# kit4b/kit4b

Hardware: AMD Instinct MI355X
Metric: Mreads/sec aligned (100 bp SE vs 3 Gbp .sfx) (higher is better)
Workload: dtype u64

## Files before the change

### kit4b_amd/csrc/k4_align.hip

```cpp
#include <stdlib.h>
#include <type_traits>
#include "k4_align_common.h"

#define K4_BS(nch) ((nch) >= 16 ? 128 : 256)
template <int NCH>
struct K4Lane {
  const uint64_t* rd;
  uint32_t* ded;
  const uint32_t* sup;
  const uint64_t* ent;
  uint64_t* memo;
  static constexpr int NW = NCH + 1;
  K4_DEV uint64_t word(int s, int c) const { return rd[(s * NW + c) * K4_BS(NCH)]; }
  K4_DEV uint64_t chunk_at(int s, int o) const {
    int w = o >> 5, sh = 2 * (o & 31);
    uint64_t hi = word(s, w);
    if (!sh) return hi;
    return (hi << sh) | (word(s, w + 1) >> (64 - sh));
  }
};

struct K4Probe {
  int cmp;
  int mm;
  int fm;
  bool exc;
};

#define K4_MEMO_NONE 0ull
K4_DEV uint64_t k4d_memo_pack(int kind, uint64_t pos, int mm, int fm) {
  return ((uint64_t)kind << 62) | ((uint64_t)(fm & 0x3FFF) << 48) | ((uint64_t)(mm & 0xFF) << 40) | (pos & 0xFFFFFFFFFFull);
}

template <int NCH>
K4_DEV K4Probe k4d_probe(const K4DevIndex& ix, const K4Lane<NCH>& ln, int s, int o, int cl, int len, uint64_t p) {
  K4Probe r;
  int64_t left = (int64_t)p - o;
  {
    const int64_t st = left < 0 ? 0 : left;
    const uint64_t b0 = (uint64_t)st >> ix.sup_shift, b1 = (uint64_t)(left + len - 1) >> ix.sup_shift;
    const uint64_t v = (((uint64_t)ln.sup[(b0 >> 5) + 1] << 32) | ln.sup[b0 >> 5]) >> (b0 & 31);
    r.exc = (v & ((2ull << (b1 - b0)) - 1ull)) != 0;
    if (r.exc && ix.sup_shift != K4_EXC_SHIFT) r.exc = k4d_any_exc(ix, left, left + len);
  }
  r.cmp = 0;
  r.mm = 0;
  r.fm = len;
  const uint32_t* wp = ix.ref2 + (left >> 4);
  uint32_t sh = (uint32_t)(left & 15) * 2;
  uint32_t wv[2 * NCH + 1];
  if (NCH <= 5 && len + 15 <= 32 * NCH) {
    uint32_t even[2 * NCH];
    k4d_load_words<2 * NCH>(wp, even);
#pragma unroll
    for (int j = 0; j < 2 * NCH + 1; j++) wv[j] = j < 2 * NCH ? even[j] : 0u;
  } else if (NCH <= 5 || len > 32 * (NCH / 2))
    k4d_load_words<2 * NCH + 1>(wp, wv);
  else {
    uint32_t half[NCH + 1];
    k4d_load_words<NCH + 1>(wp, half);
#pragma unroll
    for (int j = 0; j < 2 * NCH + 1; j++) wv[j] = j < NCH + 1 ? half[j] : 0u;
  }
  bool decided = false;
#pragma unroll
  for (int c = 0; c < NCH; c++) {
    if (32 * c < len) {
      uint64_t hi = ((uint64_t)wv[2 * c] << 32) | wv[2 * c + 1];
      uint64_t refc = sh ? (hi << sh) | (wv[2 * c + 2] >> (32 - sh)) : hi;
      uint64_t rdc = ln.word(s, c);
      uint64_t x = rdc ^ refc;
      const uint64_t xr = x & k4d_range_mask(0, len - 32 * c);
      r.mm += (int)k4d_mm_count(xr);
      if (xr && r.fm == len) r.fm = 32 * c + (__clzll(xr) >> 1);
      uint64_t cm = k4d_range_mask(o - 32 * c, o + cl - 32 * c);
      if (!decided && (x & cm)) {
        r.cmp = (rdc & cm) < (refc & cm) ? -1 : 1;
        decided = true;
      }
    }
  }
  return r;
}

template <int EL, int NCH, typename KT, bool CAPTURE>
K4_DEV int k4d_lcm_fast(const K4AlignArgs& a, const K4Lane<NCH>& ln, int len, int allow_mm, int cl, int core_delta,
                        const K4ReadParams& rp, int* p_inst, int* p_low, int* p_nxt, k4_hit* hits,
                        uint32_t& n_lookup, uint32_t& n_probe, uint32_t& n_cand, bool defer_deep = false) {
  const K4DevIndex& ix = a.ix;
  if (*p_inst > rp.max_hits && *p_low == 0) return K4_HR_HITINSTS;
  if (*p_inst >= 1 && *p_low == 0 && (*p_nxt - *p_low) < rp.mm_delta) return K4_HR_MMDELTA;
  K4State st;
  if (*p_inst <= 0 || *p_low < 0 || *p_nxt < 0) {
    st.inst = *p_inst = 0;
    st.low = *p_low = allow_mm + rp.mm_delta + 1;
    st.nxt = *p_nxt = st.low;
  } else {
    st.inst = *p_inst; st.low = *p_low; st.nxt = *p_nxt;
  }
  st.cur_hit = st.inst < rp.max_hits ? st.inst : -1;
  const int max_iter = ix.max_iter;
  const int64_t n = (int64_t)ix.n;
  const int kk = min((int)ix.k, cl);
  const int tshift = 2 * ((int)ix.k - kk);
  typedef typename std::conditional<EL == 4, uint32_t, KT>::type RT;
  constexpr uint64_t NOPOS = sizeof(RT) == 4 ? 0xFFFFFFFFull : K4_KTAB64_MASK;
  int s = rp.strand == K4_STRAND_CRICK ? 1 : 0;
  const int s_end = rp.strand == K4_STRAND_WATSON ? 0 : 1;
  bool stop = false;
  for (; s <= s_end && !stop; s++) {
    const char strand_c = s ? '-' : '+';
    int n_ded = 0;
    int cur_delta = core_delta;
    int slides = 0;
    int o_next = 0;
    bool more = true;
    bool first_group = true;
    while (more && !stop) {
      constexpr int PFN = NCH == 5 ? K4_PF5 : K4_PF;
      int oo[PFN];
      RT lb0[PFN], ps0[PFN], lb1[PFN];
      uint32_t sig[PFN];
      int cnt = 0;
#pragma unroll
      for (int j = 0; j < PFN; j++) {
        oo[j] = 0; lb0[j] = 0; ps0[j] = 0; lb1[j] = 0; sig[j] = 0;
        if (cnt == j && slides < rp.max_slides && o_next <= len - cl && cur_delta > cl / 3) {
          if (o_next + cl + cur_delta > len) cur_delta = len - (o_next + cl);
          oo[j] = o_next;
          cnt++;
          slides++;
          o_next += cur_delta;
        }
      }
      more = cnt == PFN;
      bool memo_hit = false, memo_pending = false;
      int memo_mm = 0;
#pragma unroll
      for (int j = 0; j < PFN; j++) {
        if (j < cnt) {
          if (!CAPTURE && j == 0 && first_group && tshift == 0 && (sizeof(KT) == 4 || cl >= kk + 2)) {
            const uint64_t mv = ln.memo[s * K4_BS(NCH)];
            const int kind = (int)(mv >> 62), fm = (int)((mv >> 48) & 0x3FFF), mmv = (int)((mv >> 40) & 0xFF);
            if (kind == 1 || (kind == 2 && fm < cl)) continue;
            if (kind == 2 && mmv != 0xFF) {
              lb0[0] = 0; lb1[0] = 1; ps0[0] = (RT)(mv & 0xFFFFFFFFFFull);
              memo_hit = true; memo_mm = mmv;
              continue;
            }
          }
          const uint64_t code = ln.chunk_at(s, oo[j]) >> (64 - 2 * kk);
          uint64_t sub;
          {
            KT e_lb0, e_ps0, e_lb1;
            k4d_ktab_fetch<KT>(ix, code << tshift, (code + 1) << tshift, e_lb0, e_ps0, sig[j], e_lb1, sub,
                               sizeof(KT) == 8 && tshift == 0 && cl >= kk + 2);
            lb0[j] = (RT)e_lb0; ps0[j] = (RT)e_ps0; lb1[j] = (RT)e_lb1;
          }
          if (CAPTURE && defer_deep && tshift == 0 && (uint64_t)(lb1[j] - lb0[j]) > K4_DEFER_BUCKET) return K4_DEFER;
          if (a.deep_general && (!CAPTURE || a.deep_general == 1) && tshift == 0 && (uint64_t)(lb1[j] - lb0[j]) > K4_DEFER_BUCKET) return K4_NEED_SLOW;
          if (sizeof(KT) == 8 && tshift == 0 && cl >= kk + 2 && sub != K4_KTAB64_IRREGULAR) {
            uint32_t before, count;
            k4d_ktab_sub(sub, (uint32_t)(ln.chunk_at(s, oo[j] + kk) >> 60), before, count);
            if (before) ps0[j] = (RT)NOPOS;
            lb0[j] += (RT)before;
            lb1[j] = lb0[j] + (RT)count;
          }
          if (CAPTURE && j == 0 && first_group && tshift == 0) {
            if (lb1[0] == lb0[0]) ln.memo[s * K4_BS(NCH)] = k4d_memo_pack(1, 0, 0, 0);
            else memo_pending = lb1[0] == lb0[0] + 1;
          }
          if (sizeof(KT) == 4 && tshift == 0 && lb1[j] == lb0[j] + 1 && cl > kk) {
            const int nb = min(K4_SIG_BASES32, cl - kk);
            const uint32_t cb = (uint32_t)(ln.chunk_at(s, oo[j] + kk) >> 32);
            const uint32_t df = (cb ^ sig[j]) & (0xFFFFFFFFu << (32 - 2 * nb));
            if (df) {
              lb1[j] = lb0[j];
              if (CAPTURE && j == 0 && first_group) {
                ln.memo[s * K4_BS(NCH)] = k4d_memo_pack(2, (uint64_t)ps0[0], 0xFF, kk + (__clz(df) >> 1));
                memo_pending = false;
              }
            }
          }
        }
      }
      uint32_t touch = 0;
#pragma unroll
      for (int j = 0; j < PFN; j++)
        if (j < cnt && tshift == 0 && lb1[j] > lb0[j] && !(j == 0 && memo_hit) && (sizeof(KT) == 4 || (uint64_t)ps0[j] != NOPOS))
          touch |= ix.ref2[((int64_t)ps0[j] - oo[j]) >> 4];

#pragma unroll
      for (int j = 0; j < PFN; j++) {
        if (j >= cnt || stop) continue;
        const int o = oo[j];
        n_lookup++;
        int64_t lo = (int64_t)lb0[j];
        int64_t hi = (int64_t)lb1[j] - 1;
        const int64_t bucket_hi = hi;
        int64_t found = -1;
        uint64_t fpos = 0;
        int fmm = 0;
        while (lo <= hi) {
          const int64_t mid = (lo + hi) >> 1;
          const uint64_t p = (tshift == 0 && mid == (int64_t)lb0[j] && (sizeof(KT) == 4 || (uint64_t)ps0[j] != NOPOS))
                                 ? (uint64_t)ps0[j] : k4d_sa_at<EL>(ix, (uint64_t)mid);
          K4Probe pr;
          if (!CAPTURE && j == 0 && memo_hit) { pr.cmp = 0; pr.mm = memo_mm; pr.fm = len; pr.exc = false; }
          else {
            pr = k4d_probe<NCH>(ix, ln, s, o, cl, len, p);
            n_probe++;
            if (CAPTURE && j == 0 && memo_pending) ln.memo[s * K4_BS(NCH)] = k4d_memo_pack(2, p, pr.mm > 254 ? 254 : pr.mm, pr.fm);
          }
          if (pr.exc) return K4_NEED_SLOW;
          if (pr.cmp > 0) lo = mid + 1;
          else {
            if (pr.cmp == 0) { found = mid; fpos = p; fmm = pr.mm; }
            hi = mid - 1;
          }
        }
        if (found != lo) continue;
        int64_t idx = found;
        uint64_t p = fpos;
        int mm = fmm;
        int iter = 0;
        bool first = true;
        while (!max_iter || iter < max_iter) {
          if (!first) {
            if (idx >= bucket_hi || idx + 1 >= n) break;
            const uint64_t p2 = k4d_sa_at<EL>(ix, (uint64_t)idx + 1);
            if ((int64_t)p2 + cl > n) break;
            const K4Probe pr = k4d_probe<NCH>(ix, ln, s, o, cl, len, p2);
            n_probe++;
            if (pr.exc) return K4_NEED_SLOW;
            if (pr.cmp != 0) break;
            idx += 1; p = p2; mm = pr.mm;
          }
          first = false;
          if (p < (uint64_t)o) continue;
          const uint64_t left = p - (uint64_t)o;
          int e;
          uint64_t e_start, e_end;
          if (ix.n_entries <= K4_LDS_ENTRIES) {
            int lo_e = 0, hi_e = (int)ix.n_entries - 1;
            e = -1; e_start = 0; e_end = 0;
            while (hi_e >= lo_e) {
              const int mid_e = (hi_e + lo_e) >> 1;
              const uint64_t sv = ln.ent[mid_e];
              if (sv > left) { hi_e = mid_e - 1; continue; }
              const uint64_t ev = ln.ent[K4_LDS_ENTRIES + mid_e];
              if (ev >= left) { e = mid_e; e_start = sv; e_end = ev; break; }
              lo_e = mid_e + 1;
            }
          } else {
            e = k4d_map_entry(ix, left);
            e_start = e >= 0 ? ix.ent_start[e] : 0;
            e_end = e >= 0 ? ix.ent_end[e] : 0;
          }
          if (e < 0 || left + (uint64_t)len - 1 > e_end) continue;
          const uint32_t targ_id = (uint32_t)(1 + p - (uint32_t)o);
          bool dup = false;
          for (int q = 0; q < n_ded; q++) dup |= (ln.ded[q * K4_BS(NCH)] == targ_id);
          if (dup) continue;
          if (n_ded >= K4_DEDUP_CAP) return K4_NEED_SLOW;
          ln.ded[n_ded * K4_BS(NCH)] = targ_id;
          n_ded++;
          iter++;
          n_cand++;
          if (mm > allow_mm || mm >= st.nxt) continue;
          k4d_fold(st, mm, hits, rp.max_hits, ix.ent_id[e], (uint32_t)(left - e_start), len, strand_c);
          if (st.inst > rp.max_hits && st.low == 0) break;
        }
        if (st.inst > rp.max_hits && st.low == 0) stop = true;
      }
      if (touch == 0x5A5A5A5Au && len < 0) n_probe++;
      first_group = false;
    }
  }
  return k4d_lcm_result(*p_inst, *p_low, p_nxt, st, rp.mm_delta, rp.max_hits, p_inst, p_low);
}

K4_DEV uint64_t k4d_rev2(uint64_t x) {
  uint64_t y = __brevll(x);
  return ((y & 0x5555555555555555ull) << 1) | ((y >> 1) & 0x5555555555555555ull);
}

template <int NCH>
K4_DEV uint32_t k4d_pack_read(const uint8_t* __restrict__ src, int len, uint64_t* col, uint32_t& n_ns) {
  constexpr int NW = NCH + 1;
  uint32_t fl = 0;
  n_ns = 0;
  const uint32_t sh = (uint32_t)(reinterpret_cast<uintptr_t>(src) & 3);
  const uint32_t* __restrict__ src32 = reinterpret_cast<const uint32_t*>(src - sh);
  const int span = len + (int)sh;
#pragma unroll
  for (int c = 0; c < NCH; c++) {
    uint64_t acc = 0;
    if (32 * c < len) {
      uint32_t dq[9] = {0, 0, 0, 0, 0, 0, 0, 0, 0};
      if (c * 32 + 32 <= span) {
        uint32_t d8[8];
        k4d_load_words<8>(src32 + c * 8, d8);
#pragma unroll
        for (int q = 0; q < 8; q++) dq[q] = d8[q];
      } else {
#pragma unroll
        for (int q = 0; q < 8; q++)
          if (c * 32 + q * 4 < span) dq[q] = src32[c * 8 + q];
      }
      if (c * 32 + 32 < span) dq[8] = src32[c * 8 + 8];
#pragma unroll
      for (int q = 0; q < 8; q++) {
        const int base = c * 32 + q * 4;
        uint32_t d = __builtin_amdgcn_alignbyte(dq[q + 1], dq[q], sh);
        d &= 0x07070707u;
        if (base + 4 > len) d &= len > base ? (0xFFFFFFFFu >> (8 * (4 - (len - base)))) : 0u;
        const uint32_t hi4 = d & 0x04040404u;
        if (hi4) {
          const uint32_t inval = hi4 & ((d << 1) | (d << 2)) & 0x04040404u;
          if (inval) fl |= K4_RF_INVALID;
          n_ns += __popc(hi4 & ~inval);
          d &= ~(hi4 | (hi4 >> 1) | (hi4 >> 2));
        }
        acc = (acc << 8) | ((d & 3) << 6) | (((d >> 8) & 3) << 4) | (((d >> 16) & 3) << 2) | ((d >> 24) & 3);
      }
    }
    col[c * K4_BS(NCH)] = acc;
  }
  col[NCH * K4_BS(NCH)] = 0;
  if (n_ns) fl |= K4_RF_HAS_N;
#pragma unroll
  for (int c = 0; c < NCH; c++) {
    uint64_t r = 0;
    if (32 * c < len) {
      const int o = len - 32 * (c + 1);
      uint64_t f;
      if (o >= 0) {
        const int w = o >> 5, sh = 2 * (o & 31);
        const uint64_t hi = col[w * K4_BS(NCH)];
        f = sh ? (hi << sh) | (col[(w + 1) * K4_BS(NCH)] >> (64 - sh)) : hi;
      } else
        f = col[0] >> (2 * (-o));
      r = k4d_rev2(~f) & k4d_range_mask(0, len - 32 * c);
    }
    col[(NW + c) * K4_BS(NCH)] = r;
  }
  col[(NW + NCH) * K4_BS(NCH)] = 0;
  return fl;
}

template <int EL, int NCH, bool FIRST, typename KT, bool DEFER = false>
__global__ void __launch_bounds__(K4_BS(NCH), (NCH >= 16 ? K4_STEP_WAVES_LONG : NCH >= 8 ? K4_STEP_WAVES_MID : NCH == 5 ? K4_STEP_WAVES_5 : K4_STEP_WAVES)) k4k_align_step(K4AlignArgs a, int step, const uint32_t* __restrict__ in_ids,
                                                      const uint64_t* __restrict__ in_rows,
                                                      const uint32_t* __restrict__ in_count, uint32_t* __restrict__ out_ids,
                                                      uint64_t* __restrict__ out_rows, uint32_t* __restrict__ out_count) {
  extern __shared__ uint64_t lds[];
  constexpr int NW = NCH + 1;
  const int tid = threadIdx.x;
  const int lane = tid & 63;
  K4Lane<NCH> ln;
  ln.rd = lds + tid;
  ln.ded = reinterpret_cast<uint32_t*>(lds + 2 * NW * K4_BS(NCH)) + tid;
  ln.memo = lds + 2 * NW * K4_BS(NCH) + (K4_DEDUP_CAP * K4_BS(NCH)) / 2 + tid;
  uint64_t* ent_l = lds + 2 * NW * K4_BS(NCH) + (K4_DEDUP_CAP * K4_BS(NCH)) / 2 + 2 * K4_BS(NCH);
  uint32_t* sup_l = reinterpret_cast<uint32_t*>(ent_l + 2 * K4_LDS_ENTRIES);
  ln.ent = ent_l;
  ln.sup = sup_l;
  for (int q = tid; q < K4_SUP_WORDS; q += K4_BS(NCH)) sup_l[q] = a.ix.excsup[q];
  if (a.ix.n_entries <= K4_LDS_ENTRIES)
    for (int q = tid; q < (int)a.ix.n_entries; q += K4_BS(NCH)) {
      ent_l[q] = a.ix.ent_start[q];
      ent_l[K4_LDS_ENTRIES + q] = a.ix.ent_end[q];
    }
  __syncthreads();
  uint64_t* col = lds + tid;
  uint32_t n_lookup = 0, n_probe = 0, n_cand = 0, n_slow = 0, n_bases = 0, n_done = 0;
  const int64_t count = (FIRST && !(DEFER && in_ids != nullptr)) ? a.n_reads : (int64_t)*in_count;
  const int64_t stride = (int64_t)gridDim.x * K4_BS(NCH);
  uint32_t ch_cur = 0, ch_left = 0;
  const bool from_list = !FIRST || (DEFER && in_ids != nullptr);
  const bool may_defer = DEFER && FIRST && in_ids == nullptr && a.defer_ids != nullptr;
  uint32_t dch_cur = 0, dch_left = 0;
  for (int64_t jb = (int64_t)blockIdx.x * K4_BS(NCH) + (tid & ~63); jb < count; jb += stride) {
    const int64_t j = jb + lane;
    bool active = j < count;
    int64_t i = 0;
    if (active) {
      i = from_list ? (int64_t)in_ids[j] : j;
      if (from_list && (uint32_t)i == K4_NO_READ) active = false;
    }
    bool slow = false, survive = false, deferred = false;
    int ext_from = -1;
    if (active) {
      const int len = (int)a.lens[i];
      const K4ReadParams rp = k4d_read_params(a, len);
      bool skip = false;
      if (FIRST) {
        if (!from_list) {
          n_done++;
          n_bases += (uint32_t)len;
        }
        uint32_t fl = 0, n_ns = 0;
        if (len < 1 || len > 32 * NCH || len > K4_MAX_FAST_READ_LEN) {
          fl = K4_RF_TOOLONG;
          if (a.mode == 1) {
            const uint8_t* src = a.reads + a.offs[i];
            for (int q = 0; q < len; q++) {
              uint32_t b = src[q] & 7;
              if (b == 4) n_ns++; else if (b > 4) fl |= K4_RF_INVALID;
            }
          }
        } else
          fl = k4d_pack_read<NCH>(a.reads + a.offs[i], len, col, n_ns);
        if (a.mode == 1) {
          int max_ns = 0;
          if (a.kp.max_ns) max_ns = max((len * a.kp.max_ns) / 100, a.kp.max_ns);
          if ((fl & K4_RF_INVALID) || (int)n_ns > max_ns) {
            k4_read_result r = {K4_HR_SEQERRS, 0, 0, 0, K4_NAR_NS, 0};
            a.rr[i] = r;
            if (!a.sparse_hits)
              for (int q = 0; q < a.max_hits; q++) *reinterpret_cast<uint4*>(&a.hits[i * a.max_hits + q]) = make_uint4(0, 0, 0, 0);
            skip = true;
          }
        }
        slow = fl != 0 && !skip;
        if (((a.mode == 1 && a.kp.pe_mode == 4) || a.best) && !skip) slow = true;
      } else {
        const uint64_t* row = in_rows + (int64_t)j * K4_ROW_WORDS(NCH);
        {
          const k4_u64x2_a8 mv = *reinterpret_cast<const k4_u64x2_a8*>(row + 2 * NCH);
          ln.memo[0] = mv.x; ln.memo[K4_BS(NCH)] = mv.y;
        }
        uint64_t rw[2 * NCH];
#pragma unroll
        for (int c = 0; c < NCH; c++) {
          const k4_u64x2_a8 v = *reinterpret_cast<const k4_u64x2_a8*>(row + 2 * c);
          rw[2 * c] = v.x; rw[2 * c + 1] = v.y;
        }
#pragma unroll
        for (int c = 0; c < NCH; c++) {
          col[c * K4_BS(NCH)] = rw[c];
          col[(NW + c) * K4_BS(NCH)] = rw[NCH + c];
        }
        col[NCH * K4_BS(NCH)] = 0;
        col[(NW + NCH) * K4_BS(NCH)] = 0;
      }
      if (!skip && (rp.core_len < 1 || rp.max_hits < 1 || rp.max_hits > a.max_hits)) slow = true;
      if (!skip && !slow) {
        int n_esc = 0;
        if (rp.tot_mm > 0)
          for (; n_esc <= rp.tot_mm; n_esc++)
            if (len / (n_esc + rp.mm_delta) <= rp.core_len) break;
        const bool has_final = rp.tot_mm > 0 ? n_esc <= rp.tot_mm : true;
        const int n_phases = n_esc + (has_final ? 1 : 0);
        int allow, cl, delta;
        if (step < n_esc) { allow = step; cl = len / (step + rp.mm_delta); delta = cl; }
        else { allow = rp.tot_mm; cl = rp.core_len; delta = rp.core_delta; }
        k4_hit* hits = a.hits + i * a.max_hits;
        int inst = 0, low = 0, nxt = 0;
        const uint32_t c0 = n_lookup, c1 = n_probe, c2 = n_cand;
        if (FIRST) { ln.memo[0] = K4_MEMO_NONE; ln.memo[K4_BS(NCH)] = K4_MEMO_NONE; }
        int rslt = k4d_lcm_fast<EL, NCH, KT, FIRST>(a, ln, len, allow, cl, delta, rp, &inst, &low, &nxt, hits, n_lookup, n_probe, n_cand, DEFER && may_defer);
        if (rslt == K4_NEED_SLOW) {
          slow = true;
          n_lookup = c0; n_probe = c1; n_cand = c2;
        }
        else if (DEFER && rslt == K4_DEFER) {
          deferred = true;
          n_lookup = c0; n_probe = c1; n_cand = c2;
        }
        else if (rslt == 0 && step + 1 >= n_phases && a.ext_on) { slow = true; ext_from = n_phases; }
        else if (rslt != 0 || step + 1 >= n_phases) k4d_finalize(a, i, len, rp, rslt, inst, low, nxt);
        else survive = true;
      }
      if (slow) {
        k4d_push_slow(a, i, ext_from >= 0 ? ext_from : step);
        n_slow++;
      }
    }
    if (FIRST && DEFER) {
      const unsigned long long dm = __ballot(deferred);
      const uint32_t dcnt = (uint32_t)__popcll(dm);
      if (dcnt) {
        if (dcnt > dch_left) {
          for (uint32_t q = lane; q < dch_left; q += 64) a.defer_ids[dch_cur + q] = K4_NO_READ;
          uint32_t base = 0;
          if (lane == 0) base = atomicAdd(&a.ctl[K4_CTL_DEFER], (uint32_t)K4_CHUNK);
          dch_cur = __shfl(base, 0, 64);
          dch_left = K4_CHUNK;
        }
        if (deferred) a.defer_ids[dch_cur + (uint32_t)__popcll(dm & ((1ull << lane) - 1ull))] = (uint32_t)i;
        dch_cur += dcnt;
        dch_left -= dcnt;
      }
    }
    const unsigned long long m = __ballot(survive);
    const uint32_t cnt = (uint32_t)__popcll(m);
    if (cnt) {
      if (cnt > ch_left) {
        for (uint32_t q = lane; q < ch_left; q += 64) out_ids[ch_cur + q] = K4_NO_READ;
        uint32_t base = 0;
        if (lane == 0) base = atomicAdd(out_count, (uint32_t)K4_CHUNK);
        ch_cur = __shfl(base, 0, 64);
        ch_left = K4_CHUNK;
      }
      if (survive) {
        const uint32_t slot = ch_cur + (uint32_t)__popcll(m & ((1ull << lane) - 1ull));
        out_ids[slot] = (uint32_t)i;
        uint64_t* row = out_rows + (int64_t)slot * K4_ROW_WORDS(NCH);
#pragma unroll
        for (int c = 0; c < NCH; c++) {
          k4_u64x2_a8 v;
          const int w0 = 2 * c, w1 = 2 * c + 1;
          v.x = w0 < NCH ? col[w0 * K4_BS(NCH)] : col[(NW + w0 - NCH) * K4_BS(NCH)];
          v.y = w1 < NCH ? col[w1 * K4_BS(NCH)] : col[(NW + w1 - NCH) * K4_BS(NCH)];
          *reinterpret_cast<k4_u64x2_a8*>(row + 2 * c) = v;
        }
        {
          k4_u64x2_a8 mv;
          mv.x = ln.memo[0]; mv.y = ln.memo[K4_BS(NCH)];
          *reinterpret_cast<k4_u64x2_a8*>(row + 2 * NCH) = mv;
        }
      }
      ch_cur += cnt;
      ch_left -= cnt;
    }
  }
  for (uint32_t q = lane; q < ch_left; q += 64) out_ids[ch_cur + q] = K4_NO_READ;
  if (FIRST && DEFER)
    for (uint32_t q = lane; q < dch_left; q += 64) a.defer_ids[dch_cur + q] = K4_NO_READ;
  {
    unsigned long long v[6] = {n_done, n_lookup, n_probe, n_cand, n_slow, n_bases};
#pragma unroll
    for (int q = 0; q < 6; q++) {
      unsigned long long x = v[q];
      for (int d = 32; d > 0; d >>= 1) x += __shfl_down(x, d, 64);
      if (lane == 0 && x) atomicAdd(&a.counters[q], x);
    }
  }
}

static uint32_t next_pow2(uint64_t v) {
  uint32_t p = 1;
  while (p < v) p <<= 1;
  return p;
}

static size_t k4_survivor_slots(size_t cap) {
  static_assert(K4_CHUNK * 7 >= 8 * 63, "cap / 7 must cover the abandoned chunk tails");
  return cap + cap / 7 + (size_t)2048 * 4 * K4_CHUNK + K4_CHUNK;
}

static int nch_for(int max_len) {
  if (max_len <= 128) return 4;
  if (max_len <= 160) return 5;
  if (max_len <= 256) return 8;
  return 16;
}

extern "C" int k4_reserve(k4_index* ix, int64_t max_reads, int32_t max_read_len, int32_t max_hits) {
  if (!ix || max_reads < 0 || max_read_len < 1 || max_hits < 1) return K4_ERR_PARAMS;
  if (max_read_len > K4_MAX_READ_LEN) return k4_fail(ix, K4_ERR_PARAMS, "read length %d exceeds %d", max_read_len, K4_MAX_READ_LEN);
  if (max_reads >= 0xFFFFFFF0ll) return k4_fail(ix, K4_ERR_PARAMS, "at most 2^32-16 reads per batch");
  K4_HIP(ix, hipSetDevice(ix->device));
  K4Workspace& w = ix->ws;
  bool touched = false;
  int fast_len = std::min<int>(max_read_len, K4_MAX_FAST_READ_LEN);
  if (max_reads > w.cap_reads || fast_len > w.cap_len) {
    int64_t cap = std::max<int64_t>(max_reads, w.cap_reads);
    cap = (cap + 255) / 256 * 256;
    int len = std::max(fast_len, w.cap_len);
    int nch = nch_for(len);
    touched = true;
    w.cap_reads = 0;
    w.cap_len = 0;
    const size_t slots = k4_survivor_slots((size_t)cap);
    for (int b = 0; b < 2; b++) {
      K4_HIP(ix, w.ids[b].reserve(slots * 4));
      K4_HIP(ix, w.rows[b].reserve(slots * K4_ROW_WORDS(nch) * 8));
    }
    K4_HIP(ix, w.slow_list.reserve((size_t)cap * 4));
    K4_HIP(ix, w.slow_step.reserve((size_t)cap));
    K4_HIP(ix, w.huge_list.reserve((size_t)cap * 4));
    K4_HIP(ix, w.huge_step.reserve((size_t)cap));
    w.cap_reads = cap;
    w.cap_len = len;
  }
  if (!w.ctl.p) {
    touched = true;
    K4_HIP(ix, w.ctl.reserve(K4_CTL_WORDS * 4));
    K4_HIP(ix, hipMemset(w.ctl.p, 0, K4_CTL_WORDS * 4));
  }
  uint64_t nodes = ix->d.max_iter ? std::min<uint64_t>((uint64_t)ix->d.max_iter * 48, K4_MAX_IDENT_NODES) : K4_MAX_IDENT_NODES;
  uint32_t hcap = next_pow2(std::max<uint64_t>(2 * nodes + 2, 1024));
  if (!w.slow_hash.p || hcap > w.slow_hash_cap) {
    touched = true;
    const size_t words = (size_t)K4_SLOW_WAVES * K4_SMALL_HASH + (size_t)K4_HUGE_WAVES * hcap;
    const size_t bytes = words * 8 + (size_t)(K4_SLOW_WAVES + K4_HUGE_WAVES) * 4;
    K4_HIP(ix, w.slow_hash.reserve(bytes));
    K4_HIP(ix, hipMemset(w.slow_hash.p, 0, bytes));
    w.slow_hash_cap = hcap;
  }
  w.cap_hits = std::max(w.cap_hits, max_hits);
  if (touched) K4_HIP(ix, hipDeviceSynchronize());
  return K4_OK;
}

template <int EL, int NCH, typename KT>
static int launch_steps(k4_index* ix, K4AlignArgs& a, int n_steps, hipStream_t st) {
  K4Workspace& w = ix->ws;
  uint32_t* const ids[2] = {w.ids[0].as<uint32_t>(), w.ids[1].as<uint32_t>()};
  uint64_t* const rows[2] = {w.rows[0].as<uint64_t>(), w.rows[1].as<uint64_t>()};
  uint32_t* const ctl = w.ctl.as<uint32_t>();
  const size_t lds = (size_t)2 * (NCH + 1) * K4_BS(NCH) * 8 + (size_t)K4_DEDUP_CAP * K4_BS(NCH) * 4 + (size_t)2 * K4_BS(NCH) * 8 + (size_t)2 * K4_LDS_ENTRIES * 8 +
                     (size_t)K4_SUP_WORDS * 4 + 16;
  if (lds > 48 * 1024) {
    K4_HIP(ix, hipFuncSetAttribute((const void*)k4k_align_step<EL, NCH, true, KT, false>, hipFuncAttributeMaxDynamicSharedMemorySize, (int)lds));
    K4_HIP(ix, hipFuncSetAttribute((const void*)k4k_align_step<EL, NCH, true, KT, true>, hipFuncAttributeMaxDynamicSharedMemorySize, (int)lds));
    K4_HIP(ix, hipFuncSetAttribute((const void*)k4k_align_step<EL, NCH, false, KT>, hipFuncAttributeMaxDynamicSharedMemorySize, (int)lds));
  }
  const unsigned full = 256 * 8 * (256 / K4_BS(NCH));
  const bool timed = ix->timing && ix->ev_used < 4096;
  if (timed) {
    if (ix->ev_used == ix->ev0.size()) {
      hipEvent_t e0, e1, e2;
      K4_HIP(ix, hipEventCreate(&e0));
      K4_HIP(ix, hipEventCreate(&e1));
      K4_HIP(ix, hipEventCreate(&e2));
      ix->ev0.push_back(e0);
      ix->ev1.push_back(e1);
      ix->ev2.push_back(e2);
    }
    K4_HIP(ix, hipEventRecord(ix->ev0[ix->ev_used], st));
  }
  unsigned grid0 = (unsigned)std::min<int64_t>((a.n_reads + K4_BS(NCH) - 1) / K4_BS(NCH), full);
  static const int deep_mode = getenv("K4_DEEP_TO_GENERAL") ? atoi(getenv("K4_DEEP_TO_GENERAL")) : 0;
  a.deep_general = (deep_mode && ix->deep_bucket_frac >= K4_DEFER_MIN_FRAC) ? deep_mode : 0;
  if (ix->deep_bucket_frac >= K4_DEFER_MIN_FRAC && a.deep_general != 1) {
    a.defer_ids = ids[1];
    hipLaunchKernelGGL((k4k_align_step<EL, NCH, true, KT, true>), dim3(grid0), dim3(K4_BS(NCH)), lds, st, a, 0, (const uint32_t*)nullptr,
                       (const uint64_t*)nullptr, (const uint32_t*)nullptr, ids[0], rows[0], ctl + 2);
    hipLaunchKernelGGL((k4k_align_step<EL, NCH, true, KT, true>), dim3(grid0), dim3(K4_BS(NCH)), lds, st, a, 0, (const uint32_t*)ids[1],
                       (const uint64_t*)nullptr, (const uint32_t*)(ctl + K4_CTL_DEFER), ids[0], rows[0], ctl + 2);
  } else {
    a.defer_ids = nullptr;
    hipLaunchKernelGGL((k4k_align_step<EL, NCH, true, KT, false>), dim3(grid0), dim3(K4_BS(NCH)), lds, st, a, 0, (const uint32_t*)nullptr,
                       (const uint64_t*)nullptr, (const uint32_t*)nullptr, ids[0], rows[0], ctl + 2);
  }
  for (int t = 1; t < n_steps; t++) {
    const int in = (t - 1) & 1, out = t & 1;
    hipLaunchKernelGGL((k4k_align_step<EL, NCH, false, KT>), dim3(grid0), dim3(K4_BS(NCH)), lds, st, a, t, ids[in], rows[in],
                       ctl + 2 + (t - 1), ids[out], rows[out], ctl + 2 + t);
  }
  if (timed) K4_HIP(ix, hipEventRecord(ix->ev1[ix->ev_used], st));
  return K4_OK;
}

template <int EL, typename KT>
static int launch_all(k4_index* ix, K4AlignArgs& a, int max_len, int n_steps, hipStream_t st) {
  K4Workspace& w = ix->ws;
  const int nch = nch_for(std::min(max_len, K4_MAX_FAST_READ_LEN));
  if (nch > nch_for(w.cap_len)) return k4_fail(ix, K4_ERR_INTERNAL, "workspace not reserved for read length %d", max_len);
  if (n_steps < 1 || n_steps > K4_CTL_WORDS - 4) return k4_fail(ix, K4_ERR_INTERNAL, "bad phase count %d", n_steps);
  a.slow_list = w.slow_list.as<uint32_t>();
  a.slow_step = w.slow_step.as<uint8_t>();
  a.ctl = w.ctl.as<uint32_t>();
  a.counters = ix->counters.as<unsigned long long>();
  a.huge_list = w.huge_list.as<uint32_t>();
  a.huge_step = w.huge_step.as<uint8_t>();
  a.slow_hash = w.slow_hash.as<uint64_t>();
  a.slow_hash_cap = w.slow_hash_cap;
  a.slow_gen = reinterpret_cast<uint32_t*>(a.slow_hash + (size_t)K4_SLOW_WAVES * K4_SMALL_HASH + (size_t)K4_HUGE_WAVES * w.slow_hash_cap);
  a.nw = nch + 1;
  if (a.n_reads == 0) return K4_OK;
  K4_HIP(ix, hipMemsetAsync(w.ctl.p, 0, K4_CTL_WORDS * 4, st));
  int rc;
  switch (nch) {
    case 4: rc = launch_steps<EL, 4, KT>(ix, a, n_steps, st); break;
    case 5: rc = launch_steps<EL, 5, KT>(ix, a, n_steps, st); break;
    case 8: rc = launch_steps<EL, 8, KT>(ix, a, n_steps, st); break;
    default: rc = launch_steps<EL, 16, KT>(ix, a, n_steps, st); break;
  }
  if (rc != K4_OK) return rc;
  rc = k4i_launch_general(ix, a, max_len, st);
  if (rc != K4_OK) return rc;
  if (ix->timing && ix->ev_used < ix->ev0.size() && ix->ev_used < 4096) {
    K4_HIP(ix, hipEventRecord(ix->ev2[ix->ev_used], st));
    ix->ev_used++;
  }
  K4_HIP(ix, hipGetLastError());
  return K4_OK;
}

static int run_dev(k4_index* ix, K4AlignArgs& a, int max_len, void* stream) {
  K4Workspace& w = ix->ws;
  if (a.n_reads > w.cap_reads || std::min(max_len, K4_MAX_FAST_READ_LEN) > w.cap_len || a.max_hits > w.cap_hits ||
      !w.slow_hash.p || !w.ids[0].p || !w.ids[1].p || !w.rows[0].p || !w.rows[1].p || !w.slow_list.p || !w.huge_list.p || !w.ctl.p)
    return k4_fail(ix, K4_ERR_PARAMS, "k4_reserve(%lld, %d, %d) must precede the *_dev call", (long long)a.n_reads,
                   max_len, a.max_hits);
  a.ix = ix->d;
  hipStream_t st = (hipStream_t)stream;
  {
    const int mc = a.mode == 0 ? a.ap.min_chimeric_len : a.kp.min_chimeric_len;
    const int mi = a.mode == 0 ? a.ap.micro_indel_len : a.kp.micro_indel_len;
    const int ms = a.mode == 0 ? a.ap.max_splice_junct_len : a.kp.max_splice_junct_len;
    if (mc < 0 || mi < 0 || mi > 20 || ms < 0 || (ms != 0 && (ms < 25 || ms > 100000)))
      return k4_fail(ix, K4_ERR_PARAMS, "MinChimericLen / microInDelLen (0..20) / MaxSpliceJunctLen (0, 25..100000) out of range");
    a.ext_on = (mc > 0 || mi > 0 || ms > 0) ? 1 : 0;
    if ((mi > 0 || ms > 0) && !a.seg2)
      return k4_fail(ix, K4_ERR_PARAMS, "microInDel / splice phases report two segments: use the *_ext entry points (k4_seg2 output)");
    if (a.ext_on && (a.best || (a.mode == 1 && a.kp.pe_mode == 4)))
      return k4_fail(ix, K4_ERR_PARAMS, "the optional AlignReads phases cannot be combined with LocateBestMatches (-N)");
    if (a.seg2 && a.n_reads > 0) K4_HIP(ix, hipMemsetAsync(a.seg2, 0, (size_t)a.n_reads * sizeof(k4_seg2), st));
  }
  int tot_mm = a.ap.tot_mm;
  if (a.mode == 1) {
    tot_mm = a.kp.max_subs == 0 ? 0 : std::max(1, (int)(0.5 + (max_len * a.kp.max_subs) / 100.0));
    tot_mm = std::min(tot_mm, 63);
  }
  const int n_steps = tot_mm + 1;
  if (ix->d.el == 4) return ix->d.ktab64 ? launch_all<4, uint64_t>(ix, a, max_len, n_steps, st) : launch_all<4, uint32_t>(ix, a, max_len, n_steps, st);
  return ix->d.ktab64 ? launch_all<5, uint64_t>(ix, a, max_len, n_steps, st) : launch_all<5, uint32_t>(ix, a, max_len, n_steps, st);
}

static int check_align_params(k4_index* ix, const k4_align_params* p) {
  if (!p) return K4_ERR_PARAMS;
  if (p->tot_mm < 0 || p->tot_mm > 63 || p->core_len < 1 || p->core_delta < 0 || p->max_core_slides < 1 ||
      p->mm_delta < 1 || p->strand < 0 || p->strand > 2 || p->max_hits < 1 || p->max_hits > 4096)
    return k4_fail(ix, K4_ERR_PARAMS, "AlignReads parameters out of range");
  return K4_OK;
}

extern "C" int k4_align_reads_batch_dev(k4_index* ix, const k4_align_params* p, int64_t n, int32_t max_len,
                                        const void* d_reads, const void* d_offs, const void* d_lens, void* d_rslt,
                                        void* d_inst, void* d_low, void* d_nxt, void* d_hits, void* stream) {
  return k4_align_reads_ext_batch_dev(ix, p, n, max_len, d_reads, d_offs, d_lens, d_rslt, d_inst, d_low, d_nxt, d_hits, nullptr, stream);
}
extern "C" int k4_align_reads_ext_batch_dev(k4_index* ix, const k4_align_params* p, int64_t n, int32_t max_len,
                                            const void* d_reads, const void* d_offs, const void* d_lens, void* d_rslt,
                                            void* d_inst, void* d_low, void* d_nxt, void* d_hits, void* d_seg2, void* stream) {
  if (!ix) return K4_ERR_PARAMS;
  int rc = check_align_params(ix, p);
  if (rc != K4_OK) return rc;
  if (n < 0 || (n > 0 && (!d_reads || !d_offs || !d_lens || !d_rslt || !d_inst || !d_low || !d_nxt || !d_hits)))
    return k4_fail(ix, K4_ERR_PARAMS, "null buffer");
  K4AlignArgs a;
  memset(&a, 0, sizeof(a));
  a.reads = (const uint8_t*)d_reads; a.offs = (const uint64_t*)d_offs; a.lens = (const uint32_t*)d_lens;
  a.n_reads = n; a.mode = 0; a.ap = *p;
  a.rslt = (int32_t*)d_rslt; a.inst = (int32_t*)d_inst; a.low = (int32_t*)d_low; a.nxt = (int32_t*)d_nxt;
  a.hits = (k4_hit*)d_hits; a.max_hits = p->max_hits;
  a.seg2 = (k4_seg2*)d_seg2;
  return run_dev(ix, a, max_len, stream);
}

extern "C" int k4_best_matches_batch_dev(k4_index* ix, const k4_align_params* p, int64_t n, int32_t max_len, const void* d_reads,
                                         const void* d_offs, const void* d_lens, void* d_rslt, void* d_inst, void* d_hits,
                                         void* stream) {
  if (!ix) return K4_ERR_PARAMS;
  int rc = check_align_params(ix, p);
  if (rc != K4_OK) return rc;
  if (n < 0 || (n > 0 && (!d_reads || !d_offs || !d_lens || !d_rslt || !d_inst || !d_hits))) return k4_fail(ix, K4_ERR_PARAMS, "null buffer");
  K4AlignArgs a;
  memset(&a, 0, sizeof(a));
  a.reads = (const uint8_t*)d_reads; a.offs = (const uint64_t*)d_offs; a.lens = (const uint32_t*)d_lens;
  a.n_reads = n; a.mode = 0; a.best = 1; a.ap = *p;
  a.rslt = (int32_t*)d_rslt; a.inst = (int32_t*)d_inst;
  a.hits = (k4_hit*)d_hits; a.max_hits = p->max_hits;
// ... 263 lines not shown
```

### kit4b_amd/csrc/k4_align_common.h

```cpp
#pragma once
#include <stdio.h>
#include <string.h>
#include <algorithm>
#include "k4_device.h"

#define K4_NEED_SLOW (-100)
#define K4_DEFER (-101)
#define K4_RF_HAS_N 1u
#define K4_RF_INVALID 2u
#define K4_RF_TOOLONG 4u
#ifndef K4_STEP_WAVES
#define K4_STEP_WAVES 4
#endif
#ifndef K4_STEP_WAVES_LONG
#define K4_STEP_WAVES_LONG 2
#endif
#ifndef K4_STEP_WAVES_5
#define K4_STEP_WAVES_5 4
#endif
#ifndef K4_STEP_WAVES_MID
#define K4_STEP_WAVES_MID 3
#endif
#define K4_CHUNK 512
#define K4_NO_READ 0xFFFFFFFFu
#define K4_ROW_WORDS(nch) (2 * (nch) + 2)
#ifndef K4_PF
#define K4_PF 4
#endif
#ifndef K4_PF5
#define K4_PF5 4
#endif
#ifndef K4_SLOW_WAVES_PER_EU
#define K4_SLOW_WAVES_PER_EU 4
#endif
#ifndef K4_SLOW_WAVES_PER_EU_EXT
#define K4_SLOW_WAVES_PER_EU_EXT 3
#endif
#ifndef K4_DEFER_BUCKET
#define K4_DEFER_BUCKET K4_DEEP_BUCKET
#endif
#define K4_DEFER_MIN_FRAC 0.002
#ifndef K4_SLOW_KB
#define K4_SLOW_KB 1
#endif
#ifndef K4_SLOW_WAVES
#define K4_SLOW_WAVES 8192
#endif
#define K4_SMALL_HASH 4096
#define K4_HUGE_WAVES 256
#define K4_CTL_HUGE 68
#define K4_CTL_DEFER 70
#define K4_CTL_WORDS 72

struct K4AlignArgs {
  K4DevIndex ix;
  const uint8_t* reads;
  const uint64_t* offs;
  const uint32_t* lens;
  int64_t n_reads;
  int32_t mode;
  int32_t sparse_hits;
  int32_t best;
  int32_t deep_general;
  k4_align_params ap;
  k4_kalign_params kp;
  int32_t* rslt;
  int32_t* inst;
  int32_t* low;
  int32_t* nxt;
  k4_read_result* rr;
  k4_hit* hits;
  k4_seg2* seg2;
  int32_t ext_on;
  int32_t max_hits;
  uint32_t* slow_list;
  uint8_t* slow_step;
  uint32_t* huge_list;
  uint8_t* huge_step;
  uint32_t* defer_ids;
  uint32_t* ctl;
  unsigned long long* counters;
  uint64_t* slow_hash;
  uint32_t* slow_gen;
  uint32_t slow_hash_cap;
  int32_t nw;
};

struct K4ReadParams {
  int tot_mm, core_len, core_delta, max_slides, mm_delta, strand, max_hits;
  int min_core_len, min_chimeric_len, micro_indel_len, max_splice_junct_len;
};

struct K4State {
  int inst, low, nxt, cur_hit;
};

K4_DEV K4ReadParams k4d_read_params(const K4AlignArgs& a, int len) {
  K4ReadParams p;
  if (a.mode == 0) {
    p.tot_mm = a.ap.tot_mm; p.core_len = a.ap.core_len; p.core_delta = a.ap.core_delta;
    p.max_slides = a.ap.max_core_slides; p.mm_delta = a.ap.mm_delta; p.strand = a.ap.strand;
    p.max_hits = a.ap.max_hits;
    p.min_core_len = a.ap.min_core_len; p.min_chimeric_len = a.ap.min_chimeric_len;
    p.micro_indel_len = a.ap.micro_indel_len; p.max_splice_junct_len = a.ap.max_splice_junct_len;
    return p;
  }
  int mm = a.kp.max_subs == 0 ? 0 : (int)(0.5 + (len * a.kp.max_subs) / 100.0);
  if (a.kp.max_subs != 0 && mm < 1) mm = 1;
  if (mm > 63) mm = 63;
  int cl = len / (a.kp.min_edit_dist == 1 ? mm + 1 : mm + 2);
  if (cl < a.kp.min_core_len) cl = a.kp.min_core_len;
  int sl = (a.kp.max_num_slides * len + 99) / 100;
  if (sl < 1) sl = 1;
  int cd = len / sl - 1;
  if (cd < cl) cd = cl;
  p.tot_mm = mm; p.core_len = cl; p.core_delta = cd; p.max_slides = sl;
  p.mm_delta = a.kp.min_edit_dist; p.strand = a.kp.strand; p.max_hits = a.kp.max_ml < 1 ? 1 : a.kp.max_ml;
  p.min_core_len = a.kp.min_core_len; p.min_chimeric_len = a.kp.min_chimeric_len;
  p.micro_indel_len = a.kp.micro_indel_len; p.max_splice_junct_len = a.kp.max_splice_junct_len;
  return p;
}

K4_DEV void k4d_store_hit(k4_hit* h, uint32_t chrom_id, uint32_t loci, int len, char strand, int mm, uint32_t ext = 0) {
  uint4 v;
  v.x = chrom_id;
  v.y = loci;
  v.z = (uint32_t)(len & 0xFFFF) | ((uint32_t)(uint8_t)strand << 16) | ((uint32_t)(mm & 0xFF) << 24);
  v.w = ext;
  *reinterpret_cast<uint4*>(h) = v;
}

K4_DEV void k4d_fold(K4State& st, int mm, k4_hit* hits, int max_hits, uint32_t chrom_id, uint32_t loci, int len,
                     char strand) {
  if (mm < st.low) {
    st.cur_hit = 0;
    st.inst = 1;
    st.nxt = st.low;
    st.low = mm;
    if (hits) k4d_store_hit(&hits[0], chrom_id, loci, len, strand, mm);
  } else if (mm == st.low) {
    st.inst += 1;
    if (st.cur_hit != -1 && st.inst <= max_hits) {
      st.cur_hit += 1;
      if (hits && st.cur_hit < max_hits) k4d_store_hit(&hits[st.cur_hit], chrom_id, loci, len, strand, mm);
    }
  } else if (mm < st.nxt)
    st.nxt = mm;
}

K4_DEV int k4d_lcm_result(int p_inst, int p_low, int* p_nxt, const K4State& st, int mm_delta, int max_hits,
                          int* o_inst, int* o_low) {
  if (p_low == st.low && p_inst == st.inst) {
    if (*p_nxt > st.nxt) {
      *p_nxt = st.nxt;
      if (st.nxt - p_low < mm_delta) return K4_HR_MMDELTA;
      return K4_HR_RMMDELTA;
    }
    return K4_HR_NONE;
  }
  *o_low = st.low; *o_inst = st.inst; *p_nxt = st.nxt;
  if (st.inst >= 1 && (st.nxt - st.low) < mm_delta) return K4_HR_MMDELTA;
  if (st.inst > max_hits) return K4_HR_HITINSTS;
  return K4_HR_HITS;
}

K4_DEV void k4d_finalize(const K4AlignArgs& a, int64_t i, int len, const K4ReadParams& rp, int rslt, int inst,
                         int low, int nxt) {
  k4_hit* hits = a.hits + i * a.max_hits;
  int nvalid = (rslt == K4_HR_HITS || rslt == K4_HR_MMDELTA || rslt == K4_HR_HITINSTS) ? min(inst, rp.max_hits) : 0;
  if (!a.sparse_hits)
    for (int q = nvalid; q < a.max_hits; q++) *reinterpret_cast<uint4*>(&hits[q]) = make_uint4(0, 0, 0, 0);
  if (a.mode == 0) {
    a.rslt[i] = rslt; a.inst[i] = inst;
    if (a.low) a.low[i] = low;
    if (a.nxt) a.nxt[i] = nxt;
    return;
  }
  k4_read_result r;
  if (inst > rp.max_hits) inst = rp.max_hits + 1;
  if (a.kp.pe_mode >= 3 && rslt == K4_HR_HITINSTS) { inst = rp.max_hits; rslt = K4_HR_HITS; }
  r.hit_rslt = rslt; r.inst = inst; r.low_mm = low; r.nxt_mm = nxt; r.nar = K4_NAR_NOHIT; r.num_hits = 0;
  switch (rslt) {
    case K4_HR_NONE: r.inst = 0; r.low_mm = 0; r.nxt_mm = 0; break;
    case K4_HR_HITS:
      if (a.kp.pe_mode >= 2) { r.nar = K4_NAR_ACCEPTED; r.num_hits = min(inst, rp.max_hits); }
      else if (!a.kp.pe_mode || inst == 1) { r.nar = K4_NAR_ACCEPTED; r.num_hits = 1; }
      else { r.nar = K4_NAR_MULTIALIGN; r.num_hits = inst; }
      break;
    case K4_HR_MMDELTA: r.nar = K4_NAR_MMDELTA; break;
    case K4_HR_HITINSTS: r.nar = K4_NAR_MULTIALIGN; break;
    default: break;
  }
  (void)len;
  a.rr[i] = r;
}

K4_DEV void k4d_push_slow(const K4AlignArgs& a, int64_t i, int step) {
  uint32_t slot = atomicAdd(&a.ctl[0], 1u);
  a.slow_list[slot] = (uint32_t)i;
  a.slow_step[slot] = (uint8_t)step;
}

int k4i_launch_general(k4_index* ix, K4AlignArgs& a, int max_len, hipStream_t st);
```

Before: 3084.

## Cache per-length read plans and a coarse entry index in LDS; speed up packing

Precomputes per-read-length phase plans (core length, delta, allowed mismatches, phase count) once per block into LDS for NCH 4 and 16. Each read then fetches its plan with one table load instead of recomputing the escalation loop. Adds a 256-bucket coarse index over entry starts so the entry binary search begins in a narrow range. Rewrites read packing to use squeeze and alignbit, with a slow exact repacking pass only when any N or invalid base is seen. Costs extra LDS and setup work per block. The byte-wide coarse index and the repurposed core_len field could differ from the original semantics in edge cases.

```diff
diff --git a/kit4b_amd/csrc/k4_align.hip b/kit4b_amd/csrc/k4_align.hip
--- a/kit4b_amd/csrc/k4_align.hip
+++ b/kit4b_amd/csrc/k4_align.hip
@@ -3,6 +3,9 @@
 #include "k4_align_common.h"
 
 #define K4_BS(nch) ((nch) >= 16 ? 128 : 256)
+#define K4_PLAN_IN_LDS(nch) ((nch) == 4 || (nch) == 16)
+#define K4_PLAN_BYTES(nch) (K4_PLAN_IN_LDS(nch) ? (32 * (nch) + 1) * 16 : 0)
+#define K4_CIDX_BLOCKS 256
 template <int NCH>
 struct K4Lane {
   const uint64_t* rd;
@@ -10,6 +13,8 @@
   const uint32_t* sup;
   const uint64_t* ent;
   uint64_t* memo;
+  const uint8_t* cidx;
+  uint32_t eshift;
   static constexpr int NW = NCH + 1;
   K4_DEV uint64_t word(int s, int c) const { return rd[(s * NW + c) * K4_BS(NCH)]; }
   K4_DEV uint64_t chunk_at(int s, int o) const {
@@ -242,7 +247,8 @@
           int e;
           uint64_t e_start, e_end;
           if (ix.n_entries <= K4_LDS_ENTRIES) {
-            int lo_e = 0, hi_e = (int)ix.n_entries - 1;
+            const uint32_t cb = (uint32_t)(left >> ln.eshift);
+            int lo_e = ln.cidx[cb], hi_e = ln.cidx[cb + 1];
             e = -1; e_start = 0; e_end = 0;
             while (hi_e >= lo_e) {
               const int mid_e = (hi_e + lo_e) >> 1;
@@ -285,6 +291,32 @@
   return ((y & 0x5555555555555555ull) << 1) | ((y >> 1) & 0x5555555555555555ull);
 }
 
+K4_DEV uint32_t k4d_squeeze4(uint32_t d) {
+  const uint32_t u = (d << 10) | d;
+  return (u << 20) | u;
+}
+
+K4_DEV uint64_t k4d_pack_chunk_exact(const uint32_t* __restrict__ src32, uint32_t sh, int span, int len, int c, uint32_t& fl, uint32_t& n_ns) {
+  uint64_t acc = 0;
+  uint32_t lo = c * 32 < span ? src32[c * 8] : 0u;
+#pragma unroll
+  for (int q = 0; q < 8; q++) {
+    const int base = c * 32 + q * 4;
+    const uint32_t hi = base + 4 < span ? src32[c * 8 + q + 1] : 0u;
+    uint32_t d = __builtin_amdgcn_alignbyte(hi, lo, sh);
+    lo = hi;
+    d &= 0x07070707u;
+    if (base + 4 > len) d &= len > base ? (0xFFFFFFFFu >> (8 * (4 - (len - base)))) : 0u;
+    const uint32_t hi4 = d & 0x04040404u;
+    const uint32_t inval = hi4 & ((d << 1) | (d << 2)) & 0x04040404u;
+    if (inval) fl |= K4_RF_INVALID;
+    n_ns += __popc(hi4 & ~inval);
+    d &= ~(hi4 | (hi4 >> 1) | (hi4 >> 2));
+    acc = (acc << 8) | (k4d_squeeze4(d & 0x03030303u) >> 24);
+  }
+  return acc;
+}
+
 template <int NCH>
 K4_DEV uint32_t k4d_pack_read(const uint8_t* __restrict__ src, int len, uint64_t* col, uint32_t& n_ns) {
   constexpr int NW = NCH + 1;
@@ -293,6 +325,9 @@
   const uint32_t sh = (uint32_t)(reinterpret_cast<uintptr_t>(src) & 3);
   const uint32_t* __restrict__ src32 = reinterpret_cast<const uint32_t*>(src - sh);
   const int span = len + (int)sh;
+  const int whole = len >> 2;
+  const uint32_t tail_mask = (len & 3) ? 0xFFFFFFFFu >> (8 * (4 - (len & 3))) : 0u;
+  uint32_t above = 0;
 #pragma unroll
   for (int c = 0; c < NCH; c++) {
     uint64_t acc = 0;
@@ -309,25 +344,33 @@
           if (c * 32 + q * 4 < span) dq[q] = src32[c * 8 + q];
       }
       if (c * 32 + 32 < span) dq[8] = src32[c * 8 + 8];
-#pragma unroll
-      for (int q = 0; q < 8; q++) {
-        const int base = c * 32 + q * 4;
-        uint32_t d = __builtin_amdgcn_alignbyte(dq[q + 1], dq[q], sh);
-        d &= 0x07070707u;
-        if (base + 4 > len) d &= len > base ? (0xFFFFFFFFu >> (8 * (4 - (len - base)))) : 0u;
-        const uint32_t hi4 = d & 0x04040404u;
-        if (hi4) {
-          const uint32_t inval = hi4 & ((d << 1) | (d << 2)) & 0x04040404u;
-          if (inval) fl |= K4_RF_INVALID;
-          n_ns += __popc(hi4 & ~inval);
-          d &= ~(hi4 | (hi4 >> 1) | (hi4 >> 2));
-        }
-        acc = (acc << 8) | ((d & 3) << 6) | (((d >> 8) & 3) << 4) | (((d >> 16) & 3) << 2) | ((d >> 24) & 3);
-      }
+      uint32_t half[2] = {0, 0};
+      if (c * 32 + 32 <= len) {
+#pragma unroll
+        for (int q = 0; q < 8; q++) {
+          const uint32_t d = __builtin_amdgcn_alignbyte(dq[q + 1], dq[q], sh);
+          above |= d & 0x04040404u;
+          half[q >> 2] = __builtin_amdgcn_alignbit(half[q >> 2], k4d_squeeze4(d & 0x03030303u), 24);
+        }
+      } else {
+#pragma unroll
+        for (int q = 0; q < 8; q++) {
+          const int w = c * 8 + q;
+          uint32_t d = __builtin_amdgcn_alignbyte(dq[q + 1], dq[q], sh);
+          d &= w < whole ? 0xFFFFFFFFu : w == whole ? tail_mask : 0u;
+          above |= d & 0x04040404u;
+          half[q >> 2] = __builtin_amdgcn_alignbit(half[q >> 2], k4d_squeeze4(d & 0x03030303u), 24);
+        }
+      }
+      acc = ((uint64_t)half[0] << 32) | half[1];
     }
     col[c * K4_BS(NCH)] = acc;
   }
   col[NCH * K4_BS(NCH)] = 0;
+  if (above) {
+#pragma unroll 1
+    for (int c = 0; 32 * c < len; c++) col[c * K4_BS(NCH)] = k4d_pack_chunk_exact(src32, sh, span, len, c, fl, n_ns);
+  }
   if (n_ns) fl |= K4_RF_HAS_N;
 #pragma unroll
   for (int c = 0; c < NCH; c++) {
@@ -364,15 +407,34 @@
   ln.memo = lds + 2 * NW * K4_BS(NCH) + (K4_DEDUP_CAP * K4_BS(NCH)) / 2 + tid;
   uint64_t* ent_l = lds + 2 * NW * K4_BS(NCH) + (K4_DEDUP_CAP * K4_BS(NCH)) / 2 + 2 * K4_BS(NCH);
   uint32_t* sup_l = reinterpret_cast<uint32_t*>(ent_l + 2 * K4_LDS_ENTRIES);
+  uint4* plan_l = reinterpret_cast<uint4*>(sup_l + K4_SUP_WORDS + 4);
+  uint8_t* cidx_l = reinterpret_cast<uint8_t*>(sup_l + K4_SUP_WORDS + 4) + K4_PLAN_BYTES(NCH);
   ln.ent = ent_l;
   ln.sup = sup_l;
+  ln.cidx = cidx_l;
+  ln.eshift = 0;
+  while ((a.ix.n >> ln.eshift) + 1 >= K4_CIDX_BLOCKS) ln.eshift++;
   for (int q = tid; q < K4_SUP_WORDS; q += K4_BS(NCH)) sup_l[q] = a.ix.excsup[q];
   if (a.ix.n_entries <= K4_LDS_ENTRIES)
     for (int q = tid; q < (int)a.ix.n_entries; q += K4_BS(NCH)) {
       ent_l[q] = a.ix.ent_start[q];
       ent_l[K4_LDS_ENTRIES + q] = a.ix.ent_end[q];
     }
+  if (K4_PLAN_IN_LDS(NCH))
+    for (int q = tid; q <= 32 * NCH; q += K4_BS(NCH)) plan_l[q] = k4d_plan_pack(k4d_read_plan(a, q, step));
   __syncthreads();
+  if (a.ix.n_entries <= K4_LDS_ENTRIES) {
+    for (int q = tid; q < K4_CIDX_BLOCKS; q += K4_BS(NCH)) {
+      const uint64_t t = (uint64_t)q << ln.eshift;
+      int lo_e = 0, hi_e = (int)a.ix.n_entries;
+      while (lo_e < hi_e) {
+        const int mid_e = (lo_e + hi_e) >> 1;
+        if (ent_l[mid_e] <= t) lo_e = mid_e + 1; else hi_e = mid_e;
+      }
+      cidx_l[q] = (uint8_t)(lo_e > 0 ? lo_e - 1 : 0);
+    }
+    __syncthreads();
+  }
   uint64_t* col = lds + tid;
   uint32_t n_lookup = 0, n_probe = 0, n_cand = 0, n_slow = 0, n_bases = 0, n_done = 0;
   const int64_t count = (FIRST && !(DEFER && in_ids != nullptr)) ? a.n_reads : (int64_t)*in_count;
@@ -393,7 +455,10 @@
     int ext_from = -1;
     if (active) {
       const int len = (int)a.lens[i];
-      const K4ReadParams rp = k4d_read_params(a, len);
+      uint4 pr;
+      if (K4_PLAN_IN_LDS(NCH)) pr = plan_l[(len >= 1 && len <= 32 * NCH) ? len : 0];
+      else pr = k4d_plan_pack(k4d_read_plan(a, len, step));
+      const K4ReadParams rp = k4d_plan_params(a, pr);
       bool skip = false;
       if (FIRST) {
         if (!from_list) {
@@ -445,17 +510,10 @@
         col[NCH * K4_BS(NCH)] = 0;
         col[(NW + NCH) * K4_BS(NCH)] = 0;
       }
-      if (!skip && (rp.core_len < 1 || rp.max_hits < 1 || rp.max_hits > a.max_hits)) slow = true;
+      if (!skip && ((pr.w & K4_PLAN_NO_CORE) || rp.max_hits < 1 || rp.max_hits > a.max_hits)) slow = true;
       if (!skip && !slow) {
-        int n_esc = 0;
-        if (rp.tot_mm > 0)
-          for (; n_esc <= rp.tot_mm; n_esc++)
-            if (len / (n_esc + rp.mm_delta) <= rp.core_len) break;
-        const bool has_final = rp.tot_mm > 0 ? n_esc <= rp.tot_mm : true;
-        const int n_phases = n_esc + (has_final ? 1 : 0);
-        int allow, cl, delta;
-        if (step < n_esc) { allow = step; cl = len / (step + rp.mm_delta); delta = cl; }
-        else { allow = rp.tot_mm; cl = rp.core_len; delta = rp.core_delta; }
+        const int n_phases = (int)((pr.w >> 8) & 0xFF);
+        const int allow = (int)(pr.w & 0xFF), cl = (int)pr.x, delta = (int)pr.y;
         k4_hit* hits = a.hits + i * a.max_hits;
         int inst = 0, low = 0, nxt = 0;
         const uint32_t c0 = n_lookup, c1 = n_probe, c2 = n_cand;
@@ -613,7 +671,7 @@
   uint64_t* const rows[2] = {w.rows[0].as<uint64_t>(), w.rows[1].as<uint64_t>()};
   uint32_t* const ctl = w.ctl.as<uint32_t>();
   const size_t lds = (size_t)2 * (NCH + 1) * K4_BS(NCH) * 8 + (size_t)K4_DEDUP_CAP * K4_BS(NCH) * 4 + (size_t)2 * K4_BS(NCH) * 8 + (size_t)2 * K4_LDS_ENTRIES * 8 +
-                     (size_t)K4_SUP_WORDS * 4 + 16;
+                     (size_t)K4_SUP_WORDS * 4 + 16 + (size_t)K4_PLAN_BYTES(NCH) + K4_CIDX_BLOCKS;
   if (lds > 48 * 1024) {
     K4_HIP(ix, hipFuncSetAttribute((const void*)k4k_align_step<EL, NCH, true, KT, false>, hipFuncAttributeMaxDynamicSharedMemorySize, (int)lds));
     K4_HIP(ix, hipFuncSetAttribute((const void*)k4k_align_step<EL, NCH, true, KT, true>, hipFuncAttributeMaxDynamicSharedMemorySize, (int)lds));
diff --git a/kit4b_amd/csrc/k4_align_common.h b/kit4b_amd/csrc/k4_align_common.h
--- a/kit4b_amd/csrc/k4_align_common.h
+++ b/kit4b_amd/csrc/k4_align_common.h
@@ -121,6 +121,45 @@
   return p;
 }
 
+struct K4ReadPlan {
+  int tot_mm, core_len, core_delta, max_slides;
+  int n_phases;
+  int allow, cl, delta;
+};
+K4_DEV K4ReadPlan k4d_read_plan(const K4AlignArgs& a, int len, int step) {
+  const K4ReadParams rp = k4d_read_params(a, len);
+  K4ReadPlan pl;
+  pl.tot_mm = rp.tot_mm; pl.core_len = rp.core_len; pl.core_delta = rp.core_delta; pl.max_slides = rp.max_slides;
+  int n_esc = 0;
+  if (rp.tot_mm > 0)
+    for (; n_esc <= rp.tot_mm; n_esc++)
+      if (len / (n_esc + rp.mm_delta) <= rp.core_len) break;
+  const bool has_final = rp.tot_mm > 0 ? n_esc <= rp.tot_mm : true;
+  pl.n_phases = n_esc + (has_final ? 1 : 0);
+  if (step < n_esc) { pl.allow = step; pl.cl = len / (step + rp.mm_delta); pl.delta = pl.cl; }
+  else { pl.allow = rp.tot_mm; pl.cl = rp.core_len; pl.delta = rp.core_delta; }
+  return pl;
+}
+#define K4_PLAN_NO_CORE (1u << 24)
+K4_DEV uint4 k4d_plan_pack(const K4ReadPlan& pl) {
+  return make_uint4((uint32_t)pl.cl, (uint32_t)pl.delta, (uint32_t)pl.max_slides,
+                    (uint32_t)pl.allow | ((uint32_t)pl.n_phases << 8) | ((uint32_t)pl.tot_mm << 16) | (pl.core_len < 1 ? K4_PLAN_NO_CORE : 0u));
+}
+K4_DEV K4ReadParams k4d_plan_params(const K4AlignArgs& a, const uint4& pr) {
+  K4ReadParams p;
+  p.tot_mm = (int)((pr.w >> 16) & 0xFF); p.core_len = (int)pr.x; p.core_delta = (int)pr.y; p.max_slides = (int)pr.z;
+  if (a.mode == 0) {
+    p.mm_delta = a.ap.mm_delta; p.strand = a.ap.strand; p.max_hits = a.ap.max_hits;
+    p.min_core_len = a.ap.min_core_len; p.min_chimeric_len = a.ap.min_chimeric_len;
+    p.micro_indel_len = a.ap.micro_indel_len; p.max_splice_junct_len = a.ap.max_splice_junct_len;
+  } else {
+    p.mm_delta = a.kp.min_edit_dist; p.strand = a.kp.strand; p.max_hits = a.kp.max_ml < 1 ? 1 : a.kp.max_ml;
+    p.min_core_len = a.kp.min_core_len; p.min_chimeric_len = a.kp.min_chimeric_len;
+    p.micro_indel_len = a.kp.micro_indel_len; p.max_splice_junct_len = a.kp.max_splice_junct_len;
+  }
+  return p;
+}
+
 K4_DEV void k4d_store_hit(k4_hit* h, uint32_t chrom_id, uint32_t loci, int len, char strand, int mm, uint32_t ext = 0) {
   uint4 v;
   v.x = chrom_id;
```

After: 3341 (median of 6 runs). 1.08x the previous value.
